# jank324/lynx

Measured on AMD Instinct MI355X. Metric: particle-element-steps/sec (whole node) + achieved HBM GB/s, Segment.track ParticleBeam, higher is better.
Workload: dtype f32

## Files before the change

### lynx_amd/csrc/lynx_device.hpp

```cpp
#pragma once

#include <hip/hip_runtime.h>

#include <type_traits>

#include "lynx_maps.hpp"
#include "lynx_unit_record.hpp"

namespace lynx {

typedef float lynx_f32x4 __attribute__((ext_vector_type(4)));
typedef double lynx_f64x2 __attribute__((ext_vector_type(2)));
template <typename T, bool VEC> struct VecOf { using type = T; static constexpr int width = 1; };
template <> struct VecOf<float, true> { using type = lynx_f32x4; static constexpr int width = 4; };
template <> struct VecOf<double, true> { using type = lynx_f64x2; static constexpr int width = 2; };

struct LatticeDev {
  const lynx_elem* elems;
  const lynx_step* steps;
  const int32_t* elem_step;
  const void* pool;
  int64_t batch;
  int32_t n_elems;
  int32_t n_steps;
// ... 955 lines not shown

template <typename T>
__device__ __forceinline__ void build_to_table(const LatticeDev& lat, const T* __restrict__ energy_in,
                                               T* __restrict__ steps_out, T* __restrict__ energy_out,
                                               int chunk, int merge_pairs) {
  extern __shared__ __attribute__((aligned(16))) unsigned char smem_raw[];
  T* s_steps = reinterpret_cast<T*>(smem_raw + build_scratch_bytes(chunk, sizeof(T)));
  T* s_energy = s_steps + (size_t)lat.n_steps * LYNX_STEP_STRIDE;
  const int64_t b = blockIdx.x;
  for (int i = threadIdx.x; i < lat.n_steps * LYNX_STEP_STRIDE; i += blockDim.x) s_steps[i] = T(0);
  __syncthreads();
  build_compose_sample<T>(lat, b, energy_in[b], s_steps, s_energy, smem_raw, chunk);
  table_sinphi<T>(lat, s_steps);
  if (merge_pairs) {
    for (int s = 1; s < lat.n_steps; ++s) {
      if (!steps_pair_up(lat.steps[s - 1], lat.steps[s])) continue;
      T* run = s_steps + (s - 1) * LYNX_STEP_STRIDE;
      T* cav = s_steps + s * LYNX_STEP_STRIDE;
      T v = T(0);
      if (threadIdx.x < 49) {
        const int i = threadIdx.x / 7, j = threadIdx.x - i * 7;
        double acc = (double)cav[i * 7] * (double)run[j];
#pragma unroll
        for (int k = 1; k < 7; ++k) acc = fma((double)cav[i * 7 + k], (double)run[k * 7 + j], acc);
        v = (T)acc;
      }
      T ci[4] = {T(0), T(0), T(0), T(0)};
      bool ill = false;
      if (threadIdx.x == 49) ill = cavity_entry_inverse<T>(cav[4 * 7 + 4], cav[4 * 7 + 5], cav[5 * 7 + 4], cav[5 * 7 + 5], ci);
      __syncthreads();
      if (threadIdx.x < 49) cav[threadIdx.x] = v;
      if (threadIdx.x == 49) {
#pragma unroll
        for (int q = 0; q < 4; ++q) cav[LYNX_ENTRY_OFFSET + q] = ci[q];
        cav[LYNX_FLAGS_OFFSET] = ill ? T(1) : T(0);
      }
      if (threadIdx.x >= 64 && threadIdx.x < 78) run[threadIdx.x - 64] = run[28 + (threadIdx.x - 64)];
      __syncthreads();
    }
  }
  for (int s = threadIdx.x; s < lat.n_steps; s += blockDim.x) {
    const bool ill = s_steps[s * LYNX_STEP_STRIDE + LYNX_FLAGS_OFFSET] != T(0);
    s_steps[s * LYNX_STEP_STRIDE + LYNX_FLAGS_OFFSET] = (T)(step_descriptor(lat, s, merge_pairs) | (ill ? LYNX_DESC_ILL : 0));
  }
  if (lat.n_steps > 0 && threadIdx.x == 0)
    s_steps[(lat.n_steps - 1) * LYNX_STEP_STRIDE + LYNX_ENERGY_OFFSET] = s_energy[lat.n_steps];
  __syncthreads();
  T* dst = steps_out + b * (int64_t)lat.n_steps * LYNX_STEP_STRIDE;
  for (int i = threadIdx.x; i < lat.n_steps * LYNX_STEP_STRIDE; i += blockDim.x) dst[i] = s_steps[i];
  if (energy_out && threadIdx.x == 0) energy_out[b] = s_energy[lat.n_steps];
}

template <typename T>
__global__ __launch_bounds__(256) void k_build(LatticeDev lat, const T* __restrict__ energy_in,
                                                T* __restrict__ steps_out, T* __restrict__ energy_out,
                                                int chunk, int merge_pairs) {
  build_to_table<T>(lat, energy_in, steps_out, energy_out, chunk, merge_pairs);
}

template <typename T, int BYTES>
__global__ __launch_bounds__(256) void k_build_inline(InlinePool<BYTES> , LatticeDev lat,
                                                       const T* __restrict__ energy_in, T* __restrict__ steps_out,
                                                       T* __restrict__ energy_out, int chunk, int merge_pairs) {
  build_to_table<T>(inline_pool_view(lat), energy_in, steps_out, energy_out, chunk, merge_pairs);
}


struct TrackArgs {
  int64_t n_particles;
  int32_t chunks;
  int32_t tiles_per_wg;
  int32_t fused_build;
  int32_t store;
  int32_t lds_scratch_bytes;
  int32_t build_chunk;
  int64_t in_stride;
  int32_t merged_pairs;
  int32_t n_observers;
  uint32_t tail_seq;
  int32_t tail_wg;
  unsigned int* tail_flag;
  int32_t stash_offset;
  int32_t reversed;
};

__device__ __forceinline__ void announce_tail(const TrackArgs& a) {
  if (a.tail_flag && blockIdx.x == (unsigned)a.tail_wg && threadIdx.x == 0)
    __hip_atomic_store(a.tail_flag, a.tail_seq, __ATOMIC_RELAXED, __HIP_MEMORY_SCOPE_SYSTEM);
}

__device__ __forceinline__ float uniform_value(float v) {
  return __int_as_float(__builtin_amdgcn_readfirstlane(__float_as_int(v)));
}
__device__ __forceinline__ double uniform_value(double v) { return v; }
__device__ __forceinline__ float wave_first(float v) { return uniform_value(v); }
__device__ __forceinline__ double wave_first(double v) {
  const long long bits = __double_as_longlong(v);
  const int lo = __builtin_amdgcn_readfirstlane((int)(bits & 0xffffffffll));
  const int hi = __builtin_amdgcn_readfirstlane((int)(bits >> 32));
  return __longlong_as_double(((long long)hi << 32) | (unsigned int)lo);
}

__device__ __forceinline__ double moment_slot_moved(const double* row, const double* c0, int j) {
  if (j == 6 || j >= 28) return row[j];
  const double n = row[35];
  if (j < 6) return row[j] + n * (row[28 + j] - c0[j]);
  int k = j - 7, i = 0, len = 6;
  while (k >= len) { k -= len; --len; ++i; }
  const int jj = i + k;
  const double ei = row[28 + i] - c0[i], ej = row[28 + jj] - c0[jj];
  return row[j] + ei * row[jj] + row[i] * ej + n * ei * ej;
}

template <bool FULL> struct MomentSet {
  static constexpr int N = FULL ? 21 : 8;
  __host__ __device__ static constexpr int row(int k) { return FULL ? tri_row(k) : (k < 6 ? k : (k == 6 ? 0 : 2)); }
  __host__ __device__ static constexpr int col(int k) { return FULL ? tri_col(k) : (k < 6 ? k : (k == 6 ? 1 : 3)); }
  __host__ __device__ static constexpr int slot(int k) { return 7 + tri_index(row(k), col(k)); }
  __host__ __device__ static constexpr int tri_index(int i, int j) { return i * 6 - (i * (i - 1)) / 2 + (j - i); }
  __host__ __device__ static constexpr int tri_row(int k) {
    int i = 0, len = 6;
    while (k >= len) { k -= len; --len; ++i; }
    return i;
  }
  __host__ __device__ static constexpr int tri_col(int k) {
    int i = 0, len = 6;
    while (k >= len) { k -= len; --len; ++i; }
    return i + k;
  }
};

template <typename T, bool FULL> struct MomentAcc {
  using Set = MomentSet<FULL>;
  double d[6], dd[Set::N], one, cnt;
  __device__ __forceinline__ void clear() {
#pragma unroll
    for (int i = 0; i < 6; ++i) d[i] = 0.0;
#pragma unroll
    for (int i = 0; i < Set::N; ++i) dd[i] = 0.0;
    one = 0.0;
    cnt = 0.0;
  }
  template <int K> __device__ __forceinline__ void products(const double (&e)[6]) {
    if constexpr (K < Set::N) {
      constexpr int r = Set::row(K), c = Set::col(K);
      dd[K] = fma(e[r], e[c], dd[K]);
      products<K + 1>(e);
    }
  }
  __device__ __forceinline__ void add(const T (&z)[7], const T (&shift)[6]) {
    double e[6];
#pragma unroll
    for (int i = 0; i < 6; ++i) {
      e[i] = (double)z[i] - (double)shift[i];
      d[i] += e[i];
    }
    one += (double)z[6];
    cnt += 1.0;
    products<0>(e);
  }
};

typedef float lynx_f32x4u __attribute__((ext_vector_type(4), aligned(4)));
typedef float lynx_f32x3u __attribute__((ext_vector_type(3), aligned(4)));
typedef double lynx_f64x2u __attribute__((ext_vector_type(2), aligned(8)));
typedef unsigned int lynx_u32x4 __attribute__((ext_vector_type(4)));
typedef unsigned int lynx_u32x4u __attribute__((ext_vector_type(4), aligned(4)));

__device__ __forceinline__ void load_particle(const float* p, float (&z)[7]) {
  const lynx_f32x4u a = *reinterpret_cast<const lynx_f32x4u*>(p);
  const lynx_f32x3u b = *reinterpret_cast<const lynx_f32x3u*>(p + 4);
  z[0] = a.x; z[1] = a.y; z[2] = a.z; z[3] = a.w; z[4] = b.x; z[5] = b.y; z[6] = b.z;
}
__device__ __forceinline__ void store_particle(float* p, const float (&z)[7]) {
  lynx_f32x4u a = {z[0], z[1], z[2], z[3]};
  lynx_f32x3u b = {z[4], z[5], z[6]};
  *reinterpret_cast<lynx_f32x4u*>(p) = a;
  *reinterpret_cast<lynx_f32x3u*>(p + 4) = b;
}
__device__ __forceinline__ void load_particle(const double* p, double (&z)[7]) {
  const lynx_f64x2u a = *reinterpret_cast<const lynx_f64x2u*>(p);
  const lynx_f64x2u b = *reinterpret_cast<const lynx_f64x2u*>(p + 2);
  const lynx_f64x2u c = *reinterpret_cast<const lynx_f64x2u*>(p + 4);
  z[0] = a.x; z[1] = a.y; z[2] = b.x; z[3] = b.y; z[4] = c.x; z[5] = c.y; z[6] = p[6];
}
__device__ __forceinline__ void store_particle(double* p, const double (&z)[7]) {
  lynx_f64x2u a = {z[0], z[1]}, b = {z[2], z[3]}, c = {z[4], z[5]};
  *reinterpret_cast<lynx_f64x2u*>(p) = a;
  *reinterpret_cast<lynx_f64x2u*>(p + 2) = b;
  *reinterpret_cast<lynx_f64x2u*>(p + 4) = c;
  p[6] = z[6];
}

constexpr int kWaveTileBytes = 7168;

__device__ __forceinline__ void wave_fence() { __builtin_amdgcn_fence(__ATOMIC_ACQ_REL, "wavefront"); }

__device__ __forceinline__ void wave_tile_fetch(const void* g, int lane, lynx_u32x4 (&v)[7]) {
  const lynx_u32x4u* src = reinterpret_cast<const lynx_u32x4u*>(g);
#pragma unroll
  for (int k = 0; k < 7; ++k) v[k] = src[k * 64 + lane];
}
__device__ __forceinline__ void wave_tile_store(void* g, int lane, const lynx_u32x4 (&v)[7]) {
  lynx_u32x4u* dst = reinterpret_cast<lynx_u32x4u*>(g);
#pragma unroll
  for (int k = 0; k < 7; ++k) __builtin_nontemporal_store(v[k], dst + k * 64 + lane);
}
template <typename T, int P>
__device__ __forceinline__ void wave_tile_to_particles(const lynx_u32x4 (&v)[7], unsigned char* lds, int lane,
                                                       T (&z)[P][7]) {
  static_assert(P * 7 * sizeof(T) == 112, "a lane owns 112 bytes of the tile");
  lynx_u32x4* l = reinterpret_cast<lynx_u32x4*>(lds);
  wave_fence();
#pragma unroll
  for (int k = 0; k < 7; ++k) l[k * 64 + lane] = v[k];
  wave_fence();
  lynx_u32x4 w[7];
#pragma unroll
  for (int k = 0; k < 7; ++k) w[k] = l[lane * 7 + k];
  constexpr int PER = 16 / sizeof(T);
#pragma unroll
  for (int f = 0; f < P * 7; ++f) {
    const lynx_u32x4 q = w[f / PER];
    if constexpr (sizeof(T) == 4) {
      z[f / 7][f % 7] = __uint_as_float(q[f % PER]);
    } else {
      const unsigned long long bits = ((unsigned long long)q[(f % PER) * 2 + 1] << 32) | q[(f % PER) * 2];
      z[f / 7][f % 7] = __longlong_as_double((long long)bits);
    }
  }
}
template <typename T, int P>
__device__ __forceinline__ void wave_tile_from_particles(const T (&z)[P][7], unsigned char* lds, int lane,
                                                         lynx_u32x4 (&v)[7]) {
  lynx_u32x4* l = reinterpret_cast<lynx_u32x4*>(lds);
  constexpr int PER = 16 / sizeof(T);
  lynx_u32x4 w[7];
#pragma unroll
  for (int f = 0; f < P * 7; ++f) {
    if constexpr (sizeof(T) == 4) {
      w[f / PER][f % PER] = __float_as_uint(z[f / 7][f % 7]);
    } else {
      const unsigned long long bits = (unsigned long long)__double_as_longlong(z[f / 7][f % 7]);
      w[f / PER][(f % PER) * 2] = (unsigned int)(bits & 0xffffffffull);
      w[f / PER][(f % PER) * 2 + 1] = (unsigned int)(bits >> 32);
    }
  }
  wave_fence();
#pragma unroll
  for (int k = 0; k < 7; ++k) l[lane * 7 + k] = w[k];
  wave_fence();
#pragma unroll
  for (int k = 0; k < 7; ++k) v[k] = l[k * 64 + lane];
}

template <int MOM> struct MomScratch { using type = double; };
template <> struct MomScratch<2> { using type = float; };
template <> struct MomScratch<3> { using type = float; };
constexpr int kMomSlabScalars = 4 * 29 * 65;
constexpr int kMomSlabScalarsCompact = 4 * 16 * 65;

template <typename T, int MOM, bool FULL>
struct LaneSums {
  using Set = MomentSet<FULL>;
  static constexpr int kRows = 8 + Set::N;
  MomentAcc<T, FULL> acc;
  float f_d[6], f_dd[Set::N], f_one = 0.f, f_cnt = 0.f;
  __device__ __forceinline__ void clear_f() {
#pragma unroll
    for (int k = 0; k < 6; ++k) f_d[k] = 0.f;
#pragma unroll
    for (int k = 0; k < Set::N; ++k) f_dd[k] = 0.f;
    f_one = 0.f;
  }
  __device__ __forceinline__ void init() {
    if (MOM == 1 || MOM == 2) acc.clear();
    if (MOM == 3) clear_f();
  }
  __device__ __forceinline__ void begin_iteration() {
    if (MOM == 2) clear_f();
  }
  template <int K> __device__ __forceinline__ void products(const float (&e)[6]) {
    if constexpr (K < Set::N) {
      constexpr int r = Set::row(K), c = Set::col(K);
      f_dd[K] = fmaf(e[r], e[c], f_dd[K]);
      products<K + 1>(e);
    }
  }
  __device__ __forceinline__ void add(const T (&z)[7], const T (&shift)[6]) {
    if (MOM == 1) acc.add(z, shift);
    if (MOM == 2 || MOM == 3) {
      float e[6];
#pragma unroll
      for (int k = 0; k < 6; ++k) {
        e[k] = (float)(z[k] - shift[k]);
        f_d[k] += e[k];
      }
      f_one += (float)z[6];
      products<0>(e);
      if (MOM == 2) acc.cnt += 1.0;
      else f_cnt += 1.f;
    }
  }
  __device__ __forceinline__ void end_iteration() {
    if (MOM == 2) {
#pragma unroll
      for (int k = 0; k < 6; ++k) acc.d[k] += (double)f_d[k];
#pragma unroll
      for (int k = 0; k < Set::N; ++k) acc.dd[k] += (double)f_dd[k];
      acc.one += (double)f_one;
    }
  }
  template <typename R> __device__ __forceinline__ void park(R* slab, int lane) const {
// ... 88 lines not shown
      for (int c = 0; c < 7; ++c) {
        zp[u / 2][c].x = (float)z[u][c];
        zp[u / 2][c].y = (float)z[u + 1][c];
      }
  }
  int n_obs = 0;
  for (int sidx = 0; sidx < S; ++sidx) {
    bool merged = false;
    const T* table = SCALAR_TABLE ? g_steps : s_steps;
    int desc = (int)uniform_value(table[sidx * LYNX_STEP_STRIDE + LYNX_FLAGS_OFFSET]);
    if (s_obs && (desc & LYNX_STEP_FLAG_OBSERVE)) {
#pragma unroll
      for (int u = 0; u < UNROLL; ++u) {
        double x, y;
        if constexpr (kPairs) {
          x = (u & 1) ? (double)zp[u / 2][0].y : (double)zp[u / 2][0].x;
          y = (u & 1) ? (double)zp[u / 2][2].y : (double)zp[u / 2][2].x;
        } else {
          x = (double)z[u][0];
          y = (double)z[u][2];
        }
        if (!live || (*live)[u]) {
          s_obs[(2 * n_obs + 0) * 256] += x;
          s_obs[(2 * n_obs + 1) * 256] += y;
        }
      }
      ++n_obs;
    }
    if constexpr (kPairs && SCALAR_TABLE && UNROLL == 2) {
      if (desc & LYNX_DESC_PAIR) {
        merged = true;
        ++sidx;
        desc = (int)uniform_value(table[sidx * LYNX_STEP_STRIDE + LYNX_FLAGS_OFFSET]);
      }
    }
    const int skind = (desc >> LYNX_DESC_KIND_SHIFT) & 3, sflags = desc & 0xffff;
    if constexpr (kMapInRegs) {
      T m[LYNX_STEP_SCALARS];
      if (SCALAR_TABLE) {
        const T* tab = g_steps + sidx * LYNX_STEP_STRIDE;
#pragma unroll
        for (int q = 0; q < LYNX_STEP_SCALARS; ++q) m[q] = uniform_value(tab[q]);
      } else {
        const T* tab = s_steps + sidx * LYNX_STEP_STRIDE;
#pragma unroll
        for (int q = 0; q < LYNX_STEP_SCALARS; ++q) m[q] = uniform_value(tab[q]);
      }
      if constexpr (kPairs) {
        const bool rows_form = __builtin_expect(merged && (desc & LYNX_DESC_ILL), 0);
        const int entry = !merged ? kEntryOwn : (rows_form ? kEntryStash : kEntryInverse);
#pragma unroll
        for (int h = 0; h < UNROLL / 2; ++h) {
          if (rows_form) {
            lynx_f32x2 s_in = zp[h][0] * uniform_value(g_steps[(sidx - 1) * LYNX_STEP_STRIDE]);
            lynx_f32x2 d_in = zp[h][0] * uniform_value(g_steps[(sidx - 1) * LYNX_STEP_STRIDE + 7]);
#pragma unroll
            for (int j = 1; j < 7; ++j) {
              s_in = pk_fma(zp[h][j], uniform_value(g_steps[(sidx - 1) * LYNX_STEP_STRIDE + j]), s_in);
              d_in = pk_fma(zp[h][j], uniform_value(g_steps[(sidx - 1) * LYNX_STEP_STRIDE + 7 + j]), d_in);
            }
            *reinterpret_cast<lynx_f32x4*>(stash) = lynx_f32x4{s_in.x, s_in.y, d_in.x, d_in.y};
          }
          apply_step_pair(m, skind, sflags, zp[h], entry, lynx_f32x2{0.f, 0.f}, lynx_f32x2{0.f, 0.f}, stash);
        }
      } else {
#pragma unroll
        for (int u = 0; u < UNROLL; ++u) apply_step<T>(m, skind, sflags, z[u]);
      }
    } else {
      const T* tab = s_steps + sidx * LYNX_STEP_STRIDE;
#pragma unroll
      for (int u = 0; u < UNROLL; ++u) apply_step<T>(tab, skind, sflags, z[u]);
    }
  }
  if constexpr (kPairs) {
#pragma unroll
    for (int u = 0; u < UNROLL; u += 2)
#pragma unroll
      for (int c = 0; c < 7; ++c) {
        z[u][c] = (T)zp[u / 2][c].x;
        z[u + 1][c] = (T)zp[u / 2][c].y;
      }
  }
}

template <typename T, int MOM, bool FULL, int UNROLL, bool FUSED, bool XPOSE> constexpr int track_waves_per_simd() {
  if (XPOSE) return 3;
  if (sizeof(T) == 4 && UNROLL == 2 && !FUSED && !FULL && (MOM == 0 || MOM == 3)) return 5;
  return 1;
}

template <typename T, int MOM, bool FULL, int UNROLL, bool FUSED, bool XPOSE>
__global__ __launch_bounds__(kTrackThreads, (track_waves_per_simd<T, MOM, FULL, UNROLL, FUSED, XPOSE>())) void k_track_direct(
    LatticeDev lat, TrackArgs a, const T* __restrict__ energy_in, const T* p_in, T* p_out,
    T* __restrict__ energy_out, const T* __restrict__ steps_in, double* __restrict__ partials,
    double* __restrict__ obs_partials) {
  static_assert(!XPOSE || (UNROLL * 7 * sizeof(T) == 112 && !FUSED), "XPOSE: a lane owns 112 bytes");
  extern __shared__ __attribute__((aligned(16))) unsigned char smem_raw[];
  announce_tail(a);
  unsigned char* s_scratch = smem_raw;
  T* s_steps = reinterpret_cast<T*>(smem_raw + a.lds_scratch_bytes);
  float* stash = reinterpret_cast<float*>(smem_raw + a.stash_offset) + threadIdx.x * 4;
  T* s_energy = s_steps + (size_t)lat.n_steps * LYNX_STEP_STRIDE;
  double* s_obs = reinterpret_cast<double*>(smem_raw + ((a.lds_scratch_bytes + ((size_t)lat.n_steps * (LYNX_STEP_STRIDE + 1) + 1) * sizeof(T) + 7) / 8 * 8)) + threadIdx.x;

  const int tid = threadIdx.x;
  const int wave = tid >> 6, lane = tid & 63;
  const unsigned wg = a.reversed ? gridDim.x - 1u - blockIdx.x : blockIdx.x;
  const int64_t b = wg / a.chunks;
  const int chunk = wg % a.chunks;
  const int64_t end = a.n_particles;
  const int S = lat.n_steps;
  constexpr int64_t kTile = (int64_t)kTrackThreads * UNROLL;
  constexpr int64_t kWaveSpan = 64 * UNROLL;
  const int64_t lane_first = XPOSE ? (int64_t)wave * kWaveSpan + (int64_t)lane * UNROLL : (int64_t)tid;
  constexpr int64_t kLaneStep = XPOSE ? 1 : kTrackThreads;
  unsigned char* s_wave = s_scratch + wave * kWaveTileBytes;
#define LYNX_TILE_OF(IT) ((int64_t)chunk * a.tiles_per_wg + (IT))
#define LYNX_WAVE_BASE(TILE) ((TILE)*kTile + (int64_t)wave * kWaveSpan)

  const T* src = p_in + b * a.in_stride;
  T* dst = p_out + b * end * 7;
  T zn[XPOSE ? 1 : UNROLL][7];
  lynx_u32x4 vn[XPOSE ? 7 : 1];
  {
    const int64_t tile = LYNX_TILE_OF(0);
    if constexpr (XPOSE) {
      if (LYNX_WAVE_BASE(tile) + kWaveSpan <= end) wave_tile_fetch(src + LYNX_WAVE_BASE(tile) * 7, lane, vn);
    } else {
      const int64_t i0 = tile * kTile + lane_first;
#pragma unroll
      for (int u = 0; u < UNROLL; ++u) {
        const int64_t i = i0 + (int64_t)u * kLaneStep;
        load_particle(src + (i < end ? i : (i0 < end ? i0 : 0)) * 7, zn[u]);
      }
    }
  }

  const bool one_run = (S == 1) && (lat.steps[0].kind == LYNX_STEP_RUN) && a.n_observers == 0;
  for (int k = 0; k < 2 * a.n_observers; ++k) s_obs[k * 256] = 0.0;
  constexpr bool kMapInRegs = sizeof(T) == 4;
  constexpr bool kScalarTable = !FUSED && kMapInRegs;
  const bool scalar_table = kScalarTable && S > 0;
  const T* g_steps = steps_in + b * (int64_t)S * LYNX_STEP_STRIDE;

  if (FUSED) {
    build_compose_sample<T>(lat, b, energy_in[b], s_steps, s_energy, s_scratch, a.build_chunk);
    table_sinphi<T>(lat, s_steps);
    for (int s = tid; s < S; s += kTrackThreads) s_steps[s * LYNX_STEP_STRIDE + LYNX_FLAGS_OFFSET] = (T)step_descriptor(lat, s, 0);
    __syncthreads();
    if (energy_out && chunk == 0 && tid == 0) energy_out[b] = s_energy[S];
  } else if (S > 0) {
    if (!scalar_table) load_steps_sample<T>(g_steps, S, s_steps);
    if (energy_out && chunk == 0 && tid == 0) energy_out[b] = g_steps[(S - 1) * LYNX_STEP_STRIDE + LYNX_ENERGY_OFFSET];
  }

  T m0[kMapInRegs ? 49 : 1];
  if (one_run && kMapInRegs) {
    if (scalar_table) {
#pragma unroll
      for (int i = 0; i < 49; ++i) m0[i] = uniform_value(g_steps[i]);
    } else {
#pragma unroll
      for (int i = 0; i < 49; ++i) m0[i] = uniform_value(s_steps[i]);
    }
  }

  LaneSums<T, MOM, FULL> sums;
  sums.init();
  T shift[6];
#pragma unroll
  for (int i = 0; i < 6; ++i) shift[i] = T(0);

  constexpr bool kLdsResident = XPOSE && sizeof(T) == 8;

  for (int it = 0; it < a.tiles_per_wg; ++it) {
    const int64_t tile = LYNX_TILE_OF(it);
    const int64_t i0 = tile * kTile + lane_first;
    if (XPOSE ? (LYNX_WAVE_BASE(tile) >= end) : (i0 >= end)) break;
    if (!kMapInRegs) LYNX_FORGET();
    const bool full = XPOSE && (LYNX_WAVE_BASE(tile) + kWaveSpan <= end);
    sums.begin_iteration();

    if constexpr (kLdsResident) {
      T* mine = reinterpret_cast<T*>(s_wave) + lane * (UNROLL * 7);
      if (full) {
        lynx_u32x4* l = reinterpret_cast<lynx_u32x4*>(s_wave);
        wave_fence();
#pragma unroll
        for (int k = 0; k < 7; ++k) l[k * 64 + lane] = vn[k];
        wave_fence();
      }
      if (it + 1 < a.tiles_per_wg) {
        const int64_t tn = LYNX_TILE_OF(it + 1);
        if (LYNX_WAVE_BASE(tn) + kWaveSpan <= end) wave_tile_fetch(src + LYNX_WAVE_BASE(tn) * 7, lane, vn);
      }
#pragma unroll 1
      for (int u = 0; u < UNROLL; ++u) {
        const int64_t i = i0 + u;
        T z[1][7];
        if (full) {
#pragma unroll
          for (int c = 0; c < 7; ++c) z[0][c] = mine[u * 7 + c];
        } else {
          load_particle(src + (i < end ? i : end - 1) * 7, z[0]);
        }
        if (one_run) {
          apply_step<T>(s_steps, LYNX_STEP_RUN, 0, z[0]);
        } else {
          const bool alive[1] = {i < end};
          apply_program_lane<T, 1, false>(lat, S, g_steps, s_steps, z, a.n_observers ? s_obs : nullptr, &alive);
        }
        if (MOM && it == 0 && u == 0) {
#pragma unroll
          for (int k = 0; k < 6; ++k) shift[k] = wave_first(z[0][k]);
        }
        if (i < end) {
          if (MOM) sums.add(z[0], shift);
          if (a.store) {
            if (full) {
#pragma unroll
              for (int c = 0; c < 7; ++c) mine[u * 7 + c] = z[0][c];
            } else {
              store_particle(dst + i * 7, z[0]);
            }
          }
        }
      }
      if (a.store && full) {
        lynx_u32x4 vo[7];
        const lynx_u32x4* l = reinterpret_cast<const lynx_u32x4*>(s_wave);
        wave_fence();
#pragma unroll
        for (int k = 0; k < 7; ++k) vo[k] = l[k * 64 + lane];
        wave_tile_store(dst + LYNX_WAVE_BASE(tile) * 7, lane, vo);
      }
    } else {
      T z[UNROLL][7];
      if constexpr (XPOSE) {
        if (full) {
          wave_tile_to_particles<T, UNROLL>(vn, s_wave, lane, z);
        } else {
#pragma unroll
          for (int u = 0; u < UNROLL; ++u) load_particle(src + (i0 + u < end ? i0 + u : end - 1) * 7, z[u]);
        }
        if (it + 1 < a.tiles_per_wg) {
          const int64_t tn = LYNX_TILE_OF(it + 1);
          if (LYNX_WAVE_BASE(tn) + kWaveSpan <= end) wave_tile_fetch(src + LYNX_WAVE_BASE(tn) * 7, lane, vn);
        }
      } else {
#pragma unroll
        for (int u = 0; u < UNROLL; ++u)
#pragma unroll
          for (int c = 0; c < 7; ++c) z[u][c] = zn[u][c];
        if (it + 1 < a.tiles_per_wg) {
          const int64_t j0 = LYNX_TILE_OF(it + 1) * kTile + lane_first;
#pragma unroll
          for (int u = 0; u < UNROLL; ++u) {
            const int64_t j = j0 + (int64_t)u * kLaneStep;
            load_particle(src + (j < end ? j : i0) * 7, zn[u]);
          }
        }
      }
      if (!one_run) {
        bool alive[UNROLL];
#pragma unroll
        for (int u = 0; u < UNROLL; ++u) alive[u] = i0 + (int64_t)u * kLaneStep < end;
        apply_program_lane<T, UNROLL, kScalarTable>(lat, S, g_steps, s_steps, z,
                                                    a.n_observers ? s_obs : nullptr, &alive, stash);
      }
#pragma unroll
      for (int u = 0; u < UNROLL; ++u) {
        const int64_t i = i0 + (int64_t)u * kLaneStep;
        if (one_run) {
          if (kMapInRegs) apply_step<T>(m0, LYNX_STEP_RUN, 0, z[u]);
          else apply_step<T>(s_steps, LYNX_STEP_RUN, 0, z[u]);
        }
        if (MOM && it == 0 && u == 0) {
#pragma unroll
          for (int k = 0; k < 6; ++k) shift[k] = wave_first(z[0][k]);
        }
        if (i < end) {
          if (a.store && !(XPOSE && full)) store_particle(dst + i * 7, z[u]);
          if (MOM) sums.add(z[u], shift);
        }
      }
      if constexpr (XPOSE) {
        if (a.store && full) {
          lynx_u32x4 vo[7];
          wave_tile_from_particles<T, UNROLL>(z, s_wave, lane, vo);
          wave_tile_store(dst + LYNX_WAVE_BASE(tile) * 7, lane, vo);
        }
      }
    }
    sums.end_iteration();
  }
#undef LYNX_TILE_OF
#undef LYNX_WAVE_BASE

  if (a.n_observers) {
    __syncthreads();
    if (tid < 2 * a.n_observers) {
      const double* row = s_obs - threadIdx.x + tid * 256;
      double tot = 0.0;
      for (int k = 0; k < 256; ++k) tot += row[k];
      obs_partials[((int64_t)b * a.chunks + chunk) * (2 * LYNX_MAX_OBSERVERS) + tid] = tot;
    }
  }

  if (MOM) workgroup_moment_record<T, MOM, FULL>(sums, shift, s_scratch, partials + ((int64_t)b * a.chunks + chunk) * kPartialStride);
}

constexpr int kReduceStage = 70;
constexpr int kReduceStageWide = 448;
template <int THREADS, int STAGE> constexpr size_t reduce_lds_bytes() {
  return (size_t)(STAGE + THREADS / kPartialStride + 1) * kPartialStride * sizeof(double);
}

__device__ __forceinline__ void write_moment_record(const double* s, double* dst, int tid) {
  const double n = s[35];
  if (tid < 6) {
    dst[tid] = s[28 + tid] + s[tid] / n;
  } else if (tid == 6) {
    dst[6] = s[6] / n;
  } else if (tid < 28) {
    int k = tid - 7, i = 0, row = 6;
    while (k >= row) { k -= row; --row; ++i; }
    const int j = i + k;
    const bool have = s[34] != 0.0 || i == j || (i == 0 && j == 1) || (i == 2 && j == 3);
    dst[tid] = have ? (s[tid] - s[i] * s[j] / n) / n : __longlong_as_double(0x7ff8000000000000ll);
  } else if (tid < 34) {
    dst[tid] = 0.0;
  } else if (tid == 34) {
    dst[34] = s[34];
  } else if (tid == 35) {
    dst[35] = n;
  }
}

template <bool FINAL, int THREADS, int STAGE>
__global__ __launch_bounds__(THREADS) void k_reduce_moments(const double* __restrict__ in, int rows, int rows_per_group,
                                                             int groups, double* __restrict__ out) {
  constexpr int kSets = THREADS / kPartialStride;
  static_assert(STAGE % kSets == 0, "every set takes the same number of staged rows");
  extern __shared__ __attribute__((aligned(16))) unsigned char smem_raw[];
  double* s_rows = reinterpret_cast<double*>(smem_raw);
  double* s_set = s_rows + STAGE * kPartialStride;
  double* s = s_set + kSets * kPartialStride;
  const int64_t b = blockIdx.x / groups;
  const int g = blockIdx.x % groups;
  const int tid = threadIdx.x;
  const int q = tid / kPartialStride, j = tid - q * kPartialStride;
  const int lo = g * rows_per_group;
  const int hi = (lo + rows_per_group) < rows ? (lo + rows_per_group) : rows;
  const double* src = in + (b * (int64_t)rows + lo) * kPartialStride;
  double v = 0.0;
  int mi = 0, mj = 0;
// ... 562 lines not shown
```

### lynx_amd/csrc/lynx_hip.hip

```cpp
#include <hip/hip_runtime.h>
#include <hip/hip_ext.h>
#include <rccl/rccl.h>

#include <algorithm>
#include <cstdio>
#include <cstdlib>
#include <cstring>
#include <map>
#include <mutex>
#include <string>
#include <type_traits>
#include <unordered_map>
#include <vector>

#include "lynx_device.hpp"
#include "lynx_grad.hpp"
#include "lynx_units.hpp"
#include "lynx_grad_units.hpp"
#include "lynx_trace.hpp"
#include "lynx_trace_grad.hpp"

using namespace lynx;

struct Knobs {
  int xpose = -1;
  int unroll = -1;
  int mom = -1;
  int min_tiles_per_wg = -1;
  int async_build = -1;
  int side_reduce = -1;
  int build_host_wait = -1;
  int gather_overlap = -1;
  int lanes_build_min_batch = 256;
  int piece = 8;
  int pair_levels_fused = 1;
  int fuse_max_chunks = 0;
  int merge_steps = 1;
  int reduce_wide = 0;
  int reduce_ticket = 1;
  int one_round = -1;
  int track_units = 1;
  int unit_pairs = 1;
  int bwd_units = 1;
  int bwd_merge = 1;
  int bwd_pairs = 1;
  int build_in_tail = 1;
  int small_inline = -1;
  int bwd_reuse_table = 1;
  int host_visible_records = 1;
  int alternate_order = 1;
  int inline_pool = 1;
};

static void load_knobs(Knobs* k) {
  *k = Knobs();
  const struct { const char* name; int* value; } table[] = {
      {"LYNX_XPOSE", &k->xpose}, {"LYNX_UNROLL", &k->unroll}, {"LYNX_MOM", &k->mom},
      {"LYNX_MIN_TILES_PER_WG", &k->min_tiles_per_wg}, {"LYNX_ASYNC_BUILD", &k->async_build},
      {"LYNX_SIDE_REDUCE", &k->side_reduce}, {"LYNX_BUILD_HOST_WAIT", &k->build_host_wait},
      {"LYNX_GATHER_OVERLAP", &k->gather_overlap}, {"LYNX_LANES_BUILD_MIN_BATCH", &k->lanes_build_min_batch},
      {"LYNX_PIECE", &k->piece}, {"LYNX_PAIR_LEVELS_FUSED", &k->pair_levels_fused},
      {"LYNX_FUSE_MAX_CHUNKS", &k->fuse_max_chunks}, {"LYNX_MERGE_STEPS", &k->merge_steps},
      {"LYNX_REDUCE_WIDE", &k->reduce_wide}, {"LYNX_REDUCE_TICKET", &k->reduce_ticket}, {"LYNX_TRACK_UNITS", &k->track_units}, {"LYNX_ONE_ROUND", &k->one_round}, {"LYNX_UNIT_PAIRS", &k->unit_pairs}, {"LYNX_BWD_UNITS", &k->bwd_units},
      {"LYNX_BWD_MERGE", &k->bwd_merge}, {"LYNX_BWD_PAIRS", &k->bwd_pairs}, {"LYNX_BUILD_IN_TAIL", &k->build_in_tail},
      {"LYNX_SMALL_INLINE", &k->small_inline}, {"LYNX_INLINE_POOL", &k->inline_pool}, {"LYNX_ALTERNATE_ORDER", &k->alternate_order}, {"LYNX_HOST_VISIBLE_RECORDS", &k->host_visible_records}, {"LYNX_BWD_REUSE_TABLE", &k->bwd_reuse_table}};
  for (const auto& t : table) {
    const char* v = getenv(t.name);
    if (v && *v) *t.value = atoi(v);
  }
}
static inline int knob(int value, int dflt) { return value >= 0 ? value : dflt; }

struct lynx_ctx {
  Knobs knobs;
  int device = 0;
  hipStream_t stream = nullptr;
  hipStream_t s_build = nullptr;
  static constexpr int kTableSlots = 3;
  hipEvent_t ev_built[kTableSlots] = {}, ev_streamed_own[kTableSlots] = {}, ev_mark = nullptr;
  hipEvent_t ev_streamed[kTableSlots] = {};
  bool streamed_valid[kTableSlots] = {};
  unsigned seq = 0;
  bool main_dirty = false;
  bool main_idle = true;
  bool plain_events = false;
  unsigned long_calls = 0;
  struct FwdTable {
    const lynx_lattice* lat = nullptr;
    uint64_t version = 0;
    const void* energy = nullptr;
    int slot = -1;
    int merged = 0;
    bool units = false;
    size_t energy_bytes = 0;
    unsigned seq = 0;
    bool valid = false;
    void written(const void* dst, size_t bytes) {
      const char *a = (const char*)dst, *e = (const char*)energy;
      if (valid && a < e + energy_bytes && a + bytes > e) valid = false;
    }
  } fwd_table;
  const void* main_wrote = nullptr;
  std::mutex mu;
  void wrote(const void* dst, size_t bytes) {
    if (!dst || bytes == 0) return;
    std::lock_guard<std::mutex> lock(mu);
    fwd_table.written(dst, bytes);
  }
  hipEvent_t ev_start = nullptr, ev_stop = nullptr;
  int32_t* h_status = nullptr;
  int32_t* d_status = nullptr;
  unsigned int* d_tail_flag = nullptr;
  uint32_t tail_seq = 0;
  int can_wait_value = 0;
  std::string err;
  hipDeviceProp_t prop;
  std::multimap<size_t, void*> free_blocks;
  std::unordered_map<void*, size_t> live;
  std::vector<std::pair<const char*, size_t>> host_ranges;
  void* scratch_level = nullptr;
  size_t scratch_level_bytes = 0;
  unsigned int* scratch_tickets = nullptr;
  size_t scratch_tickets_count = 0;
  void* scratch_obs = nullptr;
  size_t scratch_obs_bytes = 0;
  void* scratch_erun = nullptr;
  size_t scratch_erun_bytes = 0;
  void* scratch_esteps = nullptr;
  size_t scratch_esteps_bytes = 0;
  int32_t* d_spec_valid = nullptr;
  void* scratch_products = nullptr;
  size_t scratch_products_bytes = 0;
  void* scratch_coefs = nullptr;
  size_t scratch_coefs_bytes = 0;
  static constexpr int kTableBwd = kTableSlots, kTablePb = kTableSlots + 1, kTableTrace = kTableSlots + 2;
  void* scratch_steps[kTableSlots + 3] = {};
  size_t scratch_steps_bytes[kTableSlots + 3] = {};
  void* scratch_trace[2] = {nullptr, nullptr};
  size_t scratch_trace_bytes[2] = {0, 0};
  void* scratch_units_bwd[2] = {nullptr, nullptr};
  size_t scratch_units_bwd_bytes[2] = {0, 0};
  void* scratch_units[2 * kTableSlots] = {};
  size_t scratch_units_bytes[2 * kTableSlots] = {};
  void* scratch_grad[3] = {nullptr, nullptr, nullptr};
  size_t scratch_grad_bytes[3] = {0, 0, 0};
  ncclComm_t comm = nullptr;
  int comm_ranks = 0;
  hipStream_t s_side = nullptr;
// ... 1033 lines not shown
    return rc ? rc : launch_build_lanes<T>(ctx, lat, stream, d_energy_in, d_steps_out, d_energy_out, merge_pairs, d_units, d_extras);
  }
  int threads, chunk;
  build_shape<T>(ctx, lat, underneath, &threads, &chunk);
  const size_t lds = build_scratch_bytes(chunk, sizeof(T)) +
                     ((size_t)lat->n_steps * LYNX_STEP_STRIDE + lat->n_steps + 1) * sizeof(T);
  int rc;
  if (lat->prog_pool && ctx->knobs.inline_pool) {
    if ((size_t)lat->pool_count * sizeof(T) <= (size_t)kInlinePoolSmall) {
      if ((rc = allow_lds(ctx, k_build_inline<T, kInlinePoolSmall>, lds))) return rc;
      hipLaunchKernelGGL((k_build_inline<T, kInlinePoolSmall>), dim3((unsigned)lat->batch), dim3((unsigned)threads), lds, stream,
                         *reinterpret_cast<const InlinePool<kInlinePoolSmall>*>(&lat->h_pool), dev_view(lat),
                         (const T*)d_energy_in, (T*)d_steps_out, (T*)d_energy_out, chunk, merge_pairs);
    } else {
      if ((rc = allow_lds(ctx, k_build_inline<T, kInlinePoolLarge>, lds))) return rc;
      hipLaunchKernelGGL((k_build_inline<T, kInlinePoolLarge>), dim3((unsigned)lat->batch), dim3((unsigned)threads), lds, stream,
                         lat->h_pool, dev_view(lat), (const T*)d_energy_in, (T*)d_steps_out, (T*)d_energy_out, chunk, merge_pairs);
    }
  } else {
    if ((rc = sync_pool(ctx, lat)) || (rc = allow_lds(ctx, k_build<T>, lds))) return rc;
    hipLaunchKernelGGL(k_build<T>, dim3((unsigned)lat->batch), dim3((unsigned)threads), lds, stream, dev_view(lat),
                       (const T*)d_energy_in, (T*)d_steps_out, (T*)d_energy_out, chunk, merge_pairs);
  }
  HIP_TRY(ctx, hipGetLastError());
  if constexpr (sizeof(T) == 4) {
    if (d_units) {
      const UnitPlan& up = lat->units[merge_pairs ? 1 : 0];
      const int64_t n = lat->batch * up.n_units;
      hipLaunchKernelGGL(k_pack_units, dim3((unsigned)((n + 255) / 256)), dim3(256), 0, stream, up, lat->batch,
                         lat->n_steps, (const float*)d_steps_out, d_units, d_extras);
      HIP_TRY(ctx, hipGetLastError());
    }
  }
  return LYNX_OK;
}

int lynx_build_compose(lynx_ctx* ctx, lynx_lattice* lat, const void* d_energy_in, void* d_steps_out,
                       void* d_energy_out) {
  LYNX_NEED(ctx);
  ctx->main_idle = false;
  if (!ctx || !lat || !d_energy_in || !d_steps_out) return fail(ctx, LYNX_ERR_INVALID, "null argument");
  if (lat->batch > 0x7fffffffLL) return fail(ctx, LYNX_ERR_INVALID, "batch too large");
  HIP_TRY(ctx, use_device(ctx));
  ctx->main_dirty = true;
  const size_t es = dtype_size(lat->dtype);
  ctx->wrote(d_steps_out, (size_t)lat->batch * lat->n_steps * LYNX_STEP_STRIDE * es);
  ctx->wrote(d_energy_out, (size_t)lat->batch * es);
  return lat->dtype == LYNX_F64 ? launch_build<double>(ctx, lat, ctx->stream, d_energy_in, d_steps_out, d_energy_out)
                                : launch_build<float>(ctx, lat, ctx->stream, d_energy_in, d_steps_out, d_energy_out);
}


struct TrackPlan {
  hipEvent_t done = nullptr;
  bool full_cov;
  int unroll;
  int mom_mode;
  bool xpose;
  TrackArgs a;
  size_t lds;
  unsigned grid;
};

template <typename T>
static TrackPlan plan_track(lynx_ctx* ctx, const lynx_lattice* lat, int64_t B, int64_t N, int32_t S, bool fused,
                            bool moments, bool full_cov) {
  TrackPlan p;
  p.full_cov = full_cov;
  constexpr int P = 16 / (int)sizeof(T);
  const int64_t cus = ctx->prop.multiProcessorCount > 0 ? ctx->prop.multiProcessorCount : 256;
  const Knobs& kn = ctx->knobs;
  const int64_t target = 512 * cus;
  p.mom_mode = knob(kn.mom, sizeof(T) == 4 ? 2 : 1);
  if (sizeof(T) == 8 || p.mom_mode < 2 || p.mom_mode > 3) p.mom_mode = sizeof(T) == 4 ? 2 : 1;
  p.a.n_particles = N;
  p.a.fused_build = (fused && S > 0) ? 1 : 0;
  p.a.store = 0;
  p.a.build_chunk = 1;
  p.a.tail_flag = nullptr;
  p.a.tail_seq = 0;
  p.a.tail_wg = 0;
  p.a.stash_offset = 0;
  p.a.reversed = 0;
  const bool single_map = S == 1 && lat && lat->h_steps[0].kind == LYNX_STEP_RUN &&
                          !(lat->h_steps[0].flags & LYNX_STEP_FLAG_OBSERVE);
  p.xpose = !p.a.fused_build &&
            knob(kn.xpose, ((sizeof(T) == 8 || (single_map && !full_cov)) && N >= 8 * 64 * P) ? 1 : 0) != 0;
  int u = knob(kn.unroll, p.xpose ? P : (sizeof(T) == 4 ? (S > 1 ? 2 : 4) : 1));
  if (u != 1 && u != 2 && u != 4) u = 2;
  if (sizeof(T) == 8 && u > 2) u = 2;
  while (u > 1 && B * ((N + 256 * u - 1) / (256 * u)) < 4 * cus) u >>= 1;
  if (u != P) p.xpose = false;
  p.unroll = u;
  const int64_t tile = 256 * (int64_t)u;
  const int64_t ntiles = (N + tile - 1) / tile;
  int64_t min_tpw = std::max(1, knob(kn.min_tiles_per_wg, S > 1 ? 16 : 2));
  while (min_tpw > 1 && B * ((ntiles + min_tpw - 1) / min_tpw) < 4 * cus) --min_tpw;
  int64_t chunks = std::max<int64_t>(1, std::min<int64_t>((ntiles + min_tpw - 1) / min_tpw, (target + B - 1) / B));
  {
    const int64_t one_round = 3 * cus;
    const int cap = knob(kn.one_round, (S <= 1 && B * chunks > one_round && B * chunks <= 4 * one_round) ? 3 : 0);
    if (cap > 0) chunks = std::max<int64_t>(1, std::min<int64_t>(chunks, cap * cus / B));
  }
  int64_t tpw = (ntiles + chunks - 1) / chunks;
  chunks = (ntiles + tpw - 1) / tpw;
  p.a.chunks = (int32_t)chunks;
  p.a.tiles_per_wg = (int32_t)tpw;
  if (p.mom_mode == 2 && kn.mom < 0 && tpw * u <= 32) p.mom_mode = 3;
  if (p.mom_mode == 3 && tpw * u > 64) p.mom_mode = 2;
  size_t scratch = 4 * kPartialStride * sizeof(double);
  if (moments)
    scratch = std::max<size_t>(scratch, (size_t)(full_cov ? kMomSlabScalars : kMomSlabScalarsCompact) * (p.mom_mode >= 2 ? 4 : 8));
  if (p.xpose) scratch = std::max<size_t>(scratch, (size_t)(kTrackThreads / 64) * kWaveTileBytes);
  if (p.a.fused_build) {
    p.a.build_chunk = build_chunk(lat->n_elems, sizeof(T) == 4 ? 32 : 64);
    scratch = std::max<size_t>(scratch, build_scratch_bytes(p.a.build_chunk, sizeof(T)));
  }
  scratch = (scratch + 15) / 16 * 16;
  p.a.lds_scratch_bytes = (int32_t)scratch;
  p.a.n_observers = lat ? lat->n_observers : 0;
  p.lds = (scratch + ((size_t)S * LYNX_STEP_STRIDE + S + 1) * sizeof(T) + 7) / 8 * 8 + (size_t)2 * p.a.n_observers * 256 * sizeof(double);
  p.grid = (unsigned)(B * chunks);
  return p;
}

template <typename T, int MOM, bool FULL, int UNROLL, bool FUSED, bool XPOSE>
static int launch_direct_inst(lynx_ctx* ctx, const TrackPlan& p, const LatticeDev& lv, const void* d_energy_in,
                              const void* d_p_in, void* d_p_out, void* d_energy_out, const void* d_steps,
                              double* d_partials, double* d_obs) {
  int rc = allow_lds(ctx, k_track_direct<T, MOM, FULL, UNROLL, FUSED, XPOSE>, p.lds);
  if (rc) return rc;
  hipEvent_t e0 = nullptr, e1 = p.done;
  if (ctx->profiling) {
    HIP_TRY(ctx, hipEventCreateWithFlags(&e0, timing_event_flags(ctx)));
    HIP_TRY(ctx, hipEventCreateWithFlags(&e1, timing_event_flags(ctx)));
  }
  hipExtLaunchKernelGGL((k_track_direct<T, MOM, FULL, UNROLL, FUSED, XPOSE>), dim3(p.grid), dim3(kTrackThreads),
                        (std::uint32_t)p.lds, ctx->stream, e0, e1, 0u, lv, p.a, (const T*)d_energy_in, (const T*)d_p_in,
                        (T*)d_p_out, (T*)d_energy_out, (const T*)d_steps, d_partials, d_obs);
  HIP_TRY(ctx, hipGetLastError());
  if (ctx->profiling) ctx->prof_events.emplace_back(e0, e1);
  ctx->last_stream_stop = e1;
  return LYNX_OK;
}

#define LYNX_LAUNCH_ARGS ctx, p, lv, d_energy_in, d_p_in, d_p_out, d_energy_out, d_steps, d_partials, d_obs
#define LYNX_LAUNCH_PARAMS                                                                                     \
  lynx_ctx *ctx, const TrackPlan &p, const LatticeDev &lv, const void *d_energy_in, const void *d_p_in,        \
      void *d_p_out, void *d_energy_out, const void *d_steps, double *d_partials, double *d_obs

template <typename T, int MOM, bool FULL, int U>
static int launch_direct_mu(LYNX_LAUNCH_PARAMS) {
  if (p.a.fused_build) {
    if constexpr (U == 1) return launch_direct_inst<T, MOM, FULL, 1, true, false>(LYNX_LAUNCH_ARGS);
    else return fail(ctx, LYNX_ERR_INVALID, "fused build: one particle per lane");
  }
  if constexpr (U * 7 * sizeof(T) == 112) {
    if (p.xpose) return launch_direct_inst<T, MOM, FULL, U, false, true>(LYNX_LAUNCH_ARGS);
  }
  return launch_direct_inst<T, MOM, FULL, U, false, false>(LYNX_LAUNCH_ARGS);
}

template <typename T, int MOM, bool FULL>
static int launch_direct_m(LYNX_LAUNCH_PARAMS) {
  switch (p.unroll) {
    case 1: return launch_direct_mu<T, MOM, FULL, 1>(LYNX_LAUNCH_ARGS);
// ... 48 lines not shown
    const int32_t last = pair ? lat->h_steps[s + 1].last : st.last;
    if (pair) ++s;
    if (plan->n_units >= kMaxUnits || s > 255) return false;
    const int u = plan->n_units++;
    plan->slot[u] = (unsigned char)s;
    plan->pair[u] = pair ? 1 : 0;
    plan->cls[u] = (unsigned char)proposed_class(lat, st.first, last);
  }
  for (int u = plan->n_units; u < kMaxUnits; ++u) plan->slot[u] = plan->cls[u] = plan->pair[u] = 0;
  return plan->n_units > 0;
}

static int ensure_units_plan(lynx_ctx* ctx, lynx_lattice* lat, bool merged) {
  const int m = merged ? 1 : 0;
  if (lat->units_made[m]) return LYNX_OK;
  UnitPlan& up = lat->units[m];
  lat->units_ok[m] = plan_units(lat, merged, &up) && lat->batch * up.n_units * kUnitStride < 0x7fffffffLL;
  lat->units_made[m] = true;
  if (!lat->units_ok[m]) return LYNX_OK;
  std::vector<int32_t> code((size_t)lat->n_steps, -1);
  for (int u = 0; u < up.n_units; ++u) code[up.slot[u]] = step_unit_code(u, up.cls[u], up.pair[u]);
  int rc;
  if (!lat->d_step_unit[m] && (rc = ctx_alloc(ctx, code.size() * sizeof(int32_t), (void**)&lat->d_step_unit[m]))) return rc;
  HIP_TRY(ctx, hipStreamSynchronize(ctx->s_build));
  HIP_TRY(ctx, sync_main(ctx));
  HIP_TRY(ctx, hipMemcpy(lat->d_step_unit[m], code.data(), code.size() * sizeof(int32_t), hipMemcpyHostToDevice));
  return LYNX_OK;
}

template <int MOM, bool FULL, int PAIRS, bool PAIR_FORM = false>
static int launch_units_inst(lynx_ctx* ctx, const TrackPlan& p, int32_t U, int32_t S, const void* d_p_in, void* d_p_out,
                             void* d_energy_out, const void* d_steps, const void* d_units, const void* d_extras,
                             double* d_partials) {
  const size_t lds = units_lds_bytes((size_t)p.a.lds_scratch_bytes, U);
  auto kernel = k_track_units<MOM, FULL, PAIRS>;
  if constexpr (PAIR_FORM) kernel = k_track_unit_pairs<MOM, FULL>;
  int rc = allow_lds(ctx, kernel, lds);
  if (rc) return rc;
  hipEvent_t e0 = nullptr, e1 = p.done;
  if (ctx->profiling) {
    HIP_TRY(ctx, hipEventCreateWithFlags(&e0, timing_event_flags(ctx)));
    HIP_TRY(ctx, hipEventCreateWithFlags(&e1, timing_event_flags(ctx)));
  }
  hipExtLaunchKernelGGL(kernel, dim3(p.grid), dim3(kTrackThreads), (std::uint32_t)lds, ctx->stream, e0, e1,
                        0u, p.a, U, S, (const float*)d_p_in, (float*)d_p_out, (float*)d_energy_out, (const float*)d_steps,
                        (const float*)d_units, (const float*)d_extras, d_partials);
  HIP_TRY(ctx, hipGetLastError());
  if (ctx->profiling) ctx->prof_events.emplace_back(e0, e1);
  ctx->last_stream_stop = e1;
  return LYNX_OK;
}

static int launch_units(lynx_ctx* ctx, const TrackPlan& p, int32_t U, int32_t S, const void* d_p_in, void* d_p_out,
                        void* d_energy_out, const void* d_steps, const void* d_units, const void* d_extras,
                        double* d_partials, bool moments, bool pair_form) {
#define LYNX_UNITS_ARGS ctx, p, U, S, d_p_in, d_p_out, d_energy_out, d_steps, d_units, d_extras, d_partials
  if (pair_form)
    return moments ? launch_units_inst<3, false, 1, true>(LYNX_UNITS_ARGS) : launch_units_inst<0, false, 1, true>(LYNX_UNITS_ARGS);
  if (p.unroll == 4) {
    if (!moments) return launch_units_inst<0, false, 2>(LYNX_UNITS_ARGS);
    if (p.mom_mode == 3) return p.full_cov ? launch_units_inst<3, true, 2>(LYNX_UNITS_ARGS) : launch_units_inst<3, false, 2>(LYNX_UNITS_ARGS);
    return p.full_cov ? launch_units_inst<2, true, 2>(LYNX_UNITS_ARGS) : launch_units_inst<2, false, 2>(LYNX_UNITS_ARGS);
  }
  if (!moments) return launch_units_inst<0, false, 1>(LYNX_UNITS_ARGS);
  if (p.mom_mode == 3) return p.full_cov ? launch_units_inst<3, true, 1>(LYNX_UNITS_ARGS) : launch_units_inst<3, false, 1>(LYNX_UNITS_ARGS);
  return p.full_cov ? launch_units_inst<2, true, 1>(LYNX_UNITS_ARGS) : launch_units_inst<2, false, 1>(LYNX_UNITS_ARGS);
#undef LYNX_UNITS_ARGS
}

template <typename T>
static int track_particles_t(lynx_ctx* ctx, lynx_lattice* lat, const LatticeDev& lv, int64_t B, int64_t N,
                             const void* d_energy_in, const void* d_p_in, void* d_p_out, void* d_energy_out,
                             double* d_moments_out, int flags, double* d_observations = nullptr) {
  const int32_t S = lv.n_steps;
  const bool moments = (flags & (LYNX_TRACK_MOMENTS | LYNX_TRACK_COVARIANCE)) != 0;
  const bool full_cov = (flags & LYNX_TRACK_COVARIANCE) != 0;
  TrackPlan p = plan_track<T>(ctx, lat, B, N, S, true, moments, full_cov);
  bool fused = S > 0 && !(flags & LYNX_TRACK_TWO_KERNEL) && p.a.chunks <= ctx->knobs.fuse_max_chunks && p.unroll == 1;
  if (!fused) p = plan_track<T>(ctx, lat, B, N, S, false, moments, full_cov);
  p.a.store = d_p_out ? 1 : 0;
  const bool shared_in = (flags & LYNX_TRACK_SHARED_INPUT) != 0;
  p.a.in_stride = shared_in ? 0 : N * 7;
  p.a.merged_pairs = 0;
  const void* d_steps = nullptr;
  const void* d_units = nullptr;
  const void* d_extras = nullptr;
  int n_units = 0;
  bool use_units = false;
  bool tail = false;
  int rc;
  int slot = -1;
  bool async_build = false;
  bool short_call = false;
  ctx->wrote(d_p_out, (size_t)B * N * 7 * sizeof(T));
  ctx->wrote(d_energy_out, (size_t)B * sizeof(T));
  ctx->wrote(d_moments_out, (size_t)B * LYNX_MOMENT_STRIDE * sizeof(double));
  ctx->wrote(d_observations, lat ? (size_t)B * lat->n_observers * 2 * sizeof(double) : 0);
  if (S > 0 && !fused) {
    slot = (int)(ctx->seq++ % (unsigned)lynx_ctx::kTableSlots);
    const size_t need = (size_t)B * S * LYNX_STEP_STRIDE * sizeof(T);
    if ((rc = ensure_scratch(ctx, &ctx->scratch_steps[slot], &ctx->scratch_steps_bytes[slot], need))) return rc;
    bool has_pair = false;
    for (int32_t s = 1; s < S; ++s)
      has_pair |= lat->h_steps[s].kind == LYNX_STEP_CAVITY && lat->h_steps[s - 1].kind == LYNX_STEP_RUN &&
                  !(lat->h_steps[s - 1].flags & LYNX_STEP_FLAG_OBSERVE);
    p.a.merged_pairs = has_pair && sizeof(T) == 4 && p.unroll == 2 &&
                       !(flags & LYNX_TRACK_SEQUENTIAL_STEPS) && ctx->knobs.merge_steps;
    if (p.a.merged_pairs) {
      p.lds = (p.lds + 15) / 16 * 16;
      p.a.stash_offset = (int32_t)p.lds;
      p.lds += (size_t)kTrackThreads * 4 * sizeof(float);
    }
    const bool half_million = B * N >= (int64_t)512 << 10;
    short_call = half_million && (size_t)B * N * 7 * sizeof(T) < ((size_t)128 << 20) && !lat->has_cavity;
    bool inline_all = false;
    if (short_call && ctx->knobs.async_build < 0)
      inline_all = knob(ctx->knobs.small_inline, ctx->main_idle ? 1 : 0) != 0;
    const bool async = knob(ctx->knobs.async_build, half_million && !inline_all ? 1 : 0) != 0;
    async_build = async;
    hipStream_t bs = async ? ctx->s_build : ctx->stream;
    if (async) {
      if (ctx->streamed_valid[slot]) HIP_TRY(ctx, hipStreamWaitEvent(bs, ctx->ev_streamed[slot], 0));
      tail = ctx->can_wait_value && ctx->knobs.build_in_tail && !short_call;
      if (tail && ctx->tail_seq >= 2)
        HIP_TRY(ctx, hipStreamWaitValue32(bs, ctx->d_tail_flag, ctx->tail_seq - 1, hipStreamWaitValueGte, 0xffffffffu));
      if (ctx->main_dirty || (ctx->main_wrote && ctx->main_wrote == d_energy_in)) {
        HIP_TRY(ctx, hipEventRecord(ctx->ev_mark, ctx->stream));
        HIP_TRY(ctx, hipStreamWaitEvent(bs, ctx->ev_mark, 0));
        ctx->main_dirty = false;
        ctx->main_wrote = nullptr;
      }
    }
    float* d_units_w = nullptr;
    float* d_extras_w = nullptr;
    if constexpr (sizeof(T) == 4) {
      const int want_units = ctx->knobs.track_units;
      if (S > 1 && (p.unroll == 2 || p.unroll == 4) && !p.xpose && p.a.n_observers == 0 && want_units &&
          (uint64_t)N * 28u + ((uint64_t)1 << 20) < ((uint64_t)1 << 32)) {
        if ((rc = ensure_units_plan(ctx, lat, p.a.merged_pairs != 0))) return rc;
        use_units = lat->units_ok[p.a.merged_pairs ? 1 : 0];
      }
      if (want_units == 2 && !use_units)
        return fail(ctx, LYNX_ERR_INVALID, "LYNX_TRACK_UNITS=2: this call does not take the structured step loop");
      if (use_units) {
        const int64_t n = B * lat->units[p.a.merged_pairs ? 1 : 0].n_units;
        const int xs = lynx_ctx::kTableSlots + slot;
        if ((rc = ensure_scratch(ctx, &ctx->scratch_units[slot], &ctx->scratch_units_bytes[slot], (size_t)n * kUnitStride * sizeof(float))) ||
            (rc = ensure_scratch(ctx, &ctx->scratch_units[xs], &ctx->scratch_units_bytes[xs], (size_t)n * kUnitExtraStride * sizeof(float))))
          return rc;
        d_units = d_units_w = (float*)ctx->scratch_units[slot];
        d_extras = d_extras_w = (float*)ctx->scratch_units[xs];
        n_units = lat->units[p.a.merged_pairs ? 1 : 0].n_units;
      }
    }
    if ((rc = launch_build<T>(ctx, lat, bs, d_energy_in, ctx->scratch_steps[slot], nullptr, p.a.merged_pairs, async, d_units_w, d_extras_w)))
      return rc;
    if (async) {
      HIP_TRY(ctx, hipEventRecord(ctx->ev_built[slot], bs));
      const bool long_kernel = (size_t)B * N * 7 * sizeof(T) >= ((size_t)128 << 20);
      if (knob(ctx->knobs.build_host_wait, (lat->has_cavity || !long_kernel) ? 0 : 1)) HIP_TRY(ctx, hipEventSynchronize(ctx->ev_built[slot]));
      else HIP_TRY(ctx, hipStreamWaitEvent(ctx->stream, ctx->ev_built[slot], 0));
    }
    d_steps = ctx->scratch_steps[slot];
    std::lock_guard<std::mutex> lock(ctx->mu);
    ctx->fwd_table.lat = lat;
    ctx->fwd_table.version = lat->version;
// ... 1111 lines not shown
```

Before: 13980 billion.

## Add structured sparse-map fast path for single-map transposed tracking

```diff
diff --git a/lynx_amd/csrc/lynx_device.hpp b/lynx_amd/csrc/lynx_device.hpp
--- a/lynx_amd/csrc/lynx_device.hpp
+++ b/lynx_amd/csrc/lynx_device.hpp
@@ -1061,6 +1061,7 @@
   unsigned int* tail_flag;
   int32_t stash_offset;
   int32_t reversed;
+  int32_t single_map_classes;
 };
 
 __device__ __forceinline__ void announce_tail(const TrackArgs& a) {
@@ -1186,14 +1187,8 @@
   for (int k = 0; k < 7; ++k) __builtin_nontemporal_store(v[k], dst + k * 64 + lane);
 }
 template <typename T, int P>
-__device__ __forceinline__ void wave_tile_to_particles(const lynx_u32x4 (&v)[7], unsigned char* lds, int lane,
-                                                       T (&z)[P][7]) {
-  static_assert(P * 7 * sizeof(T) == 112, "a lane owns 112 bytes of the tile");
-  lynx_u32x4* l = reinterpret_cast<lynx_u32x4*>(lds);
-  wave_fence();
-#pragma unroll
-  for (int k = 0; k < 7; ++k) l[k * 64 + lane] = v[k];
-  wave_fence();
+__device__ __forceinline__ void wave_tile_read_particles(const unsigned char* lds, int lane, T (&z)[P][7]) {
+  const lynx_u32x4* l = reinterpret_cast<const lynx_u32x4*>(lds);
   lynx_u32x4 w[7];
 #pragma unroll
   for (int k = 0; k < 7; ++k) w[k] = l[lane * 7 + k];
@@ -1208,6 +1203,17 @@
       z[f / 7][f % 7] = __longlong_as_double((long long)bits);
     }
   }
+}
+template <typename T, int P>
+__device__ __forceinline__ void wave_tile_to_particles(const lynx_u32x4 (&v)[7], unsigned char* lds, int lane,
+                                                       T (&z)[P][7]) {
+  static_assert(P * 7 * sizeof(T) == 112, "a lane owns 112 bytes of the tile");
+  lynx_u32x4* l = reinterpret_cast<lynx_u32x4*>(lds);
+  wave_fence();
+#pragma unroll
+  for (int k = 0; k < 7; ++k) l[k * 64 + lane] = v[k];
+  wave_fence();
+  wave_tile_read_particles<T, P>(lds, lane, z);
 }
 template <typename T, int P>
 __device__ __forceinline__ void wave_tile_from_particles(const T (&z)[P][7], unsigned char* lds, int lane,
@@ -1462,6 +1468,47 @@
         z[u + 1][c] = (T)zp[u / 2][c].y;
       }
   }
+}
+
+
+constexpr uint64_t class_u_entry_mask() {
+  uint64_t mask = 0;
+  for (int k = 0; k < 16; ++k) mask |= (uint64_t)1 << unit_entry_u(k);
+  return mask;
+}
+
+__device__ __forceinline__ bool single_map_is_class_u(const float (&m)[49], float (&mu)[16]) {
+#pragma unroll
+  for (int k = 0; k < 16; ++k) mu[k] = m[unit_entry_u(k)];
+  constexpr uint64_t kIn = class_u_entry_mask();
+  unsigned outside = 0;
+  bool ok = __float_as_uint(m[48]) == 0x3f800000u;
+#pragma unroll
+  for (int q = 0; q < 48; ++q) {
+    const unsigned bits = __float_as_uint(m[q]);
+    if ((kIn >> q) & 1) ok = ok && ((bits & 0x7f800000u) != 0x7f800000u);
+    else outside |= bits & 0x7fffffffu;
+  }
+  return ok && outside == 0u;
+}
+
+template <typename T>
+__device__ __forceinline__ void apply_class_u(const T (&m)[16], T (&z)[7]) {
+  const T o0 = t_fma(z[6], m[2], t_fma(z[1], m[1], z[0] * m[0]));
+  const T o1 = t_fma(z[6], m[5], t_fma(z[1], m[4], z[0] * m[3]));
+  const T o2 = t_fma(z[6], m[8], t_fma(z[3], m[7], z[2] * m[6]));
+  const T o3 = t_fma(z[6], m[11], t_fma(z[3], m[10], z[2] * m[9]));
+  const T o4 = t_fma(z[5], m[13], z[4] * m[12]);
+  const T o5 = t_fma(z[5], m[15], z[4] * m[14]);
+  z[0] = o0; z[1] = o1; z[2] = o2; z[3] = o3; z[4] = o4; z[5] = o5;
+}
+
+template <typename T>
+__device__ __forceinline__ bool particle_not_finite(const T (&z)[7]) {
+  T acc = z[0] * T(0);
+#pragma unroll
+  for (int k = 1; k < 7; ++k) acc = t_fma(z[k], T(0), acc);
+  return acc != acc;
 }
 
 template <typename T, int MOM, bool FULL, int UNROLL, bool FUSED, bool XPOSE> constexpr int track_waves_per_simd() {
@@ -1545,6 +1592,14 @@
       for (int i = 0; i < 49; ++i) m0[i] = uniform_value(s_steps[i]);
     }
   }
+  constexpr bool kClassULoop = XPOSE && kMapInRegs;
+  bool class_u = false;
+  T mu[16] = {};
+  if constexpr (kClassULoop) {
+    if (one_run && a.single_map_classes) {
+      class_u = single_map_is_class_u(m0, mu);
+    }
+  }
 
   LaneSums<T, MOM, FULL> sums;
   sums.init();
@@ -1642,7 +1697,27 @@
           }
         }
       }
-      if (!one_run) {
+      bool dense_tile = true;
+      if constexpr (kClassULoop) {
+        if (__builtin_expect(class_u, 1)) {
+          bool bad = false;
+#pragma unroll
+          for (int u = 0; u < UNROLL; ++u) {
+            apply_class_u(mu, z[u]);
+            bad |= particle_not_finite(z[u]);
+          }
+          dense_tile = __builtin_amdgcn_ballot_w64(bad) != 0;
+          if (__builtin_expect(dense_tile, 0)) {
+            if (full) {
+              wave_tile_read_particles<T, UNROLL>(s_wave, lane, z);
+            } else {
+#pragma unroll
+              for (int u = 0; u < UNROLL; ++u) load_particle(src + (i0 + u < end ? i0 + u : end - 1) * 7, z[u]);
+            }
+          }
+        }
+      }
+      if (kClassULoop ? __builtin_expect(!one_run, 0) : !one_run) {
         bool alive[UNROLL];
 #pragma unroll
         for (int u = 0; u < UNROLL; ++u) alive[u] = i0 + (int64_t)u * kLaneStep < end;
@@ -1652,7 +1727,7 @@
 #pragma unroll
       for (int u = 0; u < UNROLL; ++u) {
         const int64_t i = i0 + (int64_t)u * kLaneStep;
-        if (one_run) {
+        if (one_run && dense_tile) {
           if (kMapInRegs) apply_step<T>(m0, LYNX_STEP_RUN, 0, z[u]);
           else apply_step<T>(s_steps, LYNX_STEP_RUN, 0, z[u]);
         }
diff --git a/lynx_amd/csrc/lynx_hip.hip b/lynx_amd/csrc/lynx_hip.hip
--- a/lynx_amd/csrc/lynx_hip.hip
+++ b/lynx_amd/csrc/lynx_hip.hip
@@ -50,6 +50,7 @@
   int host_visible_records = 1;
   int alternate_order = 1;
   int inline_pool = 1;
+  int single_map_classes = 1;
 };
 
 static void load_knobs(Knobs* k) {
@@ -63,7 +64,8 @@
       {"LYNX_FUSE_MAX_CHUNKS", &k->fuse_max_chunks}, {"LYNX_MERGE_STEPS", &k->merge_steps},
       {"LYNX_REDUCE_WIDE", &k->reduce_wide}, {"LYNX_REDUCE_TICKET", &k->reduce_ticket}, {"LYNX_TRACK_UNITS", &k->track_units}, {"LYNX_ONE_ROUND", &k->one_round}, {"LYNX_UNIT_PAIRS", &k->unit_pairs}, {"LYNX_BWD_UNITS", &k->bwd_units},
       {"LYNX_BWD_MERGE", &k->bwd_merge}, {"LYNX_BWD_PAIRS", &k->bwd_pairs}, {"LYNX_BUILD_IN_TAIL", &k->build_in_tail},
-      {"LYNX_SMALL_INLINE", &k->small_inline}, {"LYNX_INLINE_POOL", &k->inline_pool}, {"LYNX_ALTERNATE_ORDER", &k->alternate_order}, {"LYNX_HOST_VISIBLE_RECORDS", &k->host_visible_records}, {"LYNX_BWD_REUSE_TABLE", &k->bwd_reuse_table}};
+      {"LYNX_SMALL_INLINE", &k->small_inline}, {"LYNX_INLINE_POOL", &k->inline_pool}, {"LYNX_ALTERNATE_ORDER", &k->alternate_order}, {"LYNX_HOST_VISIBLE_RECORDS", &k->host_visible_records}, {"LYNX_BWD_REUSE_TABLE", &k->bwd_reuse_table},
+      {"LYNX_SINGLE_MAP_CLASSES", &k->single_map_classes}};
   for (const auto& t : table) {
     const char* v = getenv(t.name);
     if (v && *v) *t.value = atoi(v);
@@ -1263,6 +1265,7 @@
   p.a.tail_wg = 0;
   p.a.stash_offset = 0;
   p.a.reversed = 0;
+  p.a.single_map_classes = 0;
   const bool single_map = S == 1 && lat && lat->h_steps[0].kind == LYNX_STEP_RUN &&
                           !(lat->h_steps[0].flags & LYNX_STEP_FLAG_OBSERVE);
   p.xpose = !p.a.fused_build &&
@@ -1477,6 +1480,14 @@
   const bool shared_in = (flags & LYNX_TRACK_SHARED_INPUT) != 0;
   p.a.in_stride = shared_in ? 0 : N * 7;
   p.a.merged_pairs = 0;
+  if constexpr (sizeof(T) == 4) {
+    const bool single_run = S == 1 && lat && lat->h_steps[0].kind == LYNX_STEP_RUN && p.a.n_observers == 0;
+    const int want = ctx->knobs.single_map_classes;
+    if (single_run && p.xpose && !fused && want) p.a.single_map_classes = 1;
+    if (single_run && want == 2 &&
+        !(p.a.single_map_classes && proposed_class(lat, lat->h_steps[0].first, lat->h_steps[0].last) == kClassU))
+      return fail(ctx, LYNX_ERR_INVALID, "LYNX_SINGLE_MAP_CLASSES=2: this call does not take the structured single-map loop");
+  }
   const void* d_steps = nullptr;
   const void* d_units = nullptr;
   const void* d_extras = nullptr;
```

Result: slower. 12490 billion (-10.6%).
